# kuleshov-group/caduceus

Measured on AMD Instinct MI355X. Metric: DNA tokens/sec (whole node), hg38-style MLM pre-train step, higher is better.
Workload: dtype bf16; 1 GPU; Caduceus-PS d_model=256 n_layer=16 seqlen=131072 rcps=true MLM fwd+bwd+allreduce+AdamW, 1 seq/GPU; global_batch=1, accumulate_grad_batches=1, seq_len=131072, parallelism=dp1, params=7725312

## Files before the change

caduceus_amd/_lib.py:

```python
from __future__ import annotations

import ctypes as C
import os
import threading

import torch

HERE = os.path.dirname(os.path.abspath(__file__))
LIB_PATH = os.environ.get("CADUCEUS_AMD_LIB") or os.path.join(HERE, "libcaduceus_hip.so")

CAD_F32, CAD_BF16, CAD_F16 = 0, 1, 2
PROF_KINDS = ("scan_fwd", "scan_bwd", "conv_fwd", "conv_bwd", "add_norm_fwd", "add_norm_bwd", "embed", "lm_head", "proj")

_p = C.c_void_p
_i64 = C.c_int64
_i = C.c_int
_f = C.c_float


class EmbedArgs(C.Structure):
    _fields_ = [("ids", _p), ("comp", _p), ("weight", _p), ("out", _p), ("B", _i64), ("L", _i64), ("D", _i), ("V", _i),
                ("n_strands", _i), ("w_dtype", _i), ("out_dtype", _i)]


# ... 4 lines not shown

class AddNormArgs(C.Structure):
    _fields_ = [("x", _p), ("residual_in", _p), ("weight", _p), ("bias", _p), ("y", _p), ("residual_out", _p),
                ("rstd", _p), ("mean", _p), ("rows_per_strand", _i64), ("n_strands", _i), ("D", _i), ("eps", _f),
                ("is_rms", _i), ("swap_flip", _i), ("x_dtype", _i), ("y_dtype", _i), ("y_fp8", _p), ("y_scale", _p)]


class AddNormBwdArgs(C.Structure):
    _fields_ = [("dy", _p), ("dres_out", _p), ("sum_saved", _p), ("rstd", _p), ("mean", _p), ("weight", _p),
                ("dx", _p), ("dres_in", _p), ("dweight", _p), ("dbias", _p), ("rows_per_strand", _i64),
                ("n_strands", _i), ("D", _i), ("is_rms", _i), ("swap_flip", _i), ("x_dtype", _i), ("y_dtype", _i)]


class Conv1dArgs(C.Structure):
    _fields_ = [("x", _p), ("w", _p), ("bias", _p), ("out", _p), ("SB", _i64), ("L", _i64), ("split", _i64),
                ("E", _i), ("K", _i), ("rev_lo", _i), ("rev_hi", _i), ("dtype", _i)]


class ReduceJob(C.Structure):
    _fields_ = [("src", _p), ("dst", _p)]


class ProjTmArgs(C.Structure):
    _fields_ = [("W", _p), ("X", _p), ("X2", _p), ("out", _p), ("T", _i64), ("M", _i), ("K", _i), ("ldw", _i64), ("ldx", _i64),
                ("ldo", _i64)]


class GemmStreamArgs(C.Structure):
    _fields_ = [("A", _p), ("B", _p), ("out", _p), ("R", _i64), ("C", _i64), ("K", _i64), ("lda", _i64), ("ldb", _i64), ("ldo", _i64),
                ("nslices", _i), ("mode", _i), ("col_fastest", _i)]


class FoldF32Job(C.Structure):
    _fields_ = [("src", _p), ("dst", _p), ("n", _i64), ("stride", _i64), ("stride2", _i64), ("nparts", _i), ("nparts2", _i)]


class GemmF32Args(C.Structure):
    _fields_ = [("A", _p), ("B", _p), ("D", _p), ("addend", _p), ("M", _i64), ("N", _i64), ("K", _i64),
                ("a_rs", _i64), ("a_cs", _i64), ("b_rs", _i64), ("b_cs", _i64), ("d_rs", _i64), ("d_cs", _i64),
                ("batch", _i64), ("a_bs", _i64), ("b_bs", _i64), ("d_bs", _i64)]


class Conv1dBwdArgs(C.Structure):
    _fields_ = [("x", _p), ("w", _p), ("bias", _p), ("dout", _p), ("dx", _p), ("dw", _p), ("dbias", _p),
                ("SB", _i64), ("L", _i64), ("split", _i64), ("E", _i), ("K", _i), ("rev_lo", _i), ("rev_hi", _i),
                ("dtype", _i), ("accumulate", _i)]


class ScanArgs(C.Structure):
    _fields_ = [("u", _p), ("delta", _p), ("A", _p), ("Bm", _p), ("Cm", _p), ("D", _p), ("z", _p),
                ("delta_bias", _p), ("out", _p), ("chunk_state", _p), ("SB", _i64), ("L", _i64), ("split", _i64),
                ("E", _i), ("N", _i), ("rev_lo", _i), ("rev_hi", _i), ("dtype", _i), ("h0", _p), ("hT", _p),
                ("sum_dt", _p), ("delta_is_dt", _i), ("map_only", _i)]


class ScanBwdArgs(C.Structure):
    _fields_ = [("u", _p), ("delta", _p), ("A", _p), ("Bm", _p), ("Cm", _p), ("D", _p), ("z", _p),
                ("delta_bias", _p), ("dout", _p), ("out", _p), ("chunk_state", _p), ("du", _p), ("ddelta", _p), ("dz", _p),
                ("dA", _p), ("dB", _p), ("dC", _p), ("dD", _p), ("ddelta_bias", _p), ("SB", _i64), ("L", _i64),
                ("split", _i64), ("E", _i), ("N", _i), ("rev_lo", _i), ("rev_hi", _i), ("dtype", _i),
                ("n_partials", _i), ("dhT", _p), ("dh0", _p), ("out2", _p), ("gate_fix_list", _p), ("gate_fix_count", _p),
                ("gate_fix_dz", _p), ("delta_is_dt", _i), ("carry_only", _i), ("fold_counters", _p)]


class FoldArgs(C.Structure):
    _fields_ = [("dB_slots", _p), ("dC_slots", _p), ("dB", _p), ("dC", _p), ("counters", _p), ("abort_from", _p), ("SB", _i64),
                ("L", _i64), ("split", _i64), ("N", _i), ("n_partials", _i), ("rev_lo", _i), ("rev_hi", _i), ("dtype", _i)]
# ... 274 lines not shown
```

caduceus_amd/csrc/gemm.hip:

```cpp
#include "cad_common.h"
#include "cad_stream.h"

namespace {

#define GP_WAVES 8

template <typename TE>
__device__ __forceinline__ float gp_softplus(float x) {
    if constexpr (cad_is_bf16<TE>::value)
        return cad_softplus_lowp(x);
    else
        return cad_softplus(x);
}

#define GP_MB16 2
#define GP_NT16 32
#define GP_XFB16 1
template <int KS>
struct GpCfg {
    static constexpr int MB = KS >= 16 ? GP_MB16 : 4;
    static constexpr int MW = 16 * MB;
    static constexpr int MWG = MW * GP_WAVES;
    static constexpr int NT = KS >= 16 ? GP_NT16 : 64;
    static constexpr int ROWB = KS * 64;
// ... 1039 lines not shown
#endif

template <typename TE>
static int gemm_stream(const cad_gemm_stream_args* a, void* stream) {
    CAD_CHECK_ARG(a && a->A && a->B && a->out && (a->mode == CAD_GEMM_PARTIALS || a->mode == CAD_GEMM_OUT_T_BF16));
    if (!cad_gemm_stream_supported(a->R, a->C, a->K, a->nslices)) return CAD_ERR_UNSUPPORTED;
    CAD_CHECK_ARG(a->lda >= a->K && a->ldb >= a->C && (a->lda % 8) == 0 && (a->ldb % 8) == 0);
    CAD_CHECK_ARG((((uintptr_t)a->A | (uintptr_t)a->B) % 16) == 0);
    CAD_CHECK_ARG(a->mode == CAD_GEMM_PARTIALS || (a->nslices == 1 && a->ldo >= a->R && (a->ldo % 4) == 0 && ((uintptr_t)a->out % 8) == 0));
    CadProfScope prof(8, stream);
    const int64_t nitems = (a->R / GsCfg::RT) * (a->C / GsCfg::CT) * a->nslices;
    int64_t gx = cad_cu_count();
    if (gx > nitems) gx = nitems;
    dim3 grid((unsigned)gx), block(64 * GP_WAVES);
    if (a->mode == CAD_GEMM_PARTIALS) {
        GP_BIG_LDS((gemm_stream_kernel<CAD_GEMM_PARTIALS, TE>), GsCfg::LDS);
        CAD_LAUNCH((gemm_stream_kernel<CAD_GEMM_PARTIALS, TE>), grid, block, GsCfg::LDS, stream, *a);
    } else {
        GP_BIG_LDS((gemm_stream_kernel<CAD_GEMM_OUT_T_BF16, TE>), GsCfg::LDS);
        CAD_LAUNCH((gemm_stream_kernel<CAD_GEMM_OUT_T_BF16, TE>), grid, block, GsCfg::LDS, stream, *a);
    }
    return cad_after_launch();
}
#ifndef CAD_GEMM_TEMPLATES_ONLY
extern "C" int cad_gemm_stream(const cad_gemm_stream_args* a, void* stream) { return gemm_stream<bf16_t>(a, stream); }
#endif

#ifndef CAD_GEMM_TEMPLATES_ONLY
namespace {
struct FoldF32Jobs {
    cad_fold_f32_job j[CAD_FOLD_F32_MAX_JOBS];
    int first_block[CAD_FOLD_F32_MAX_JOBS + 1];
    int njobs;
};
#define FF_THREADS 256
__global__ __launch_bounds__(FF_THREADS) void fold_f32_multi_kernel(FoldF32Jobs jobs) {
    int ji = 0;
    while (ji + 1 < jobs.njobs && (int)blockIdx.x >= jobs.first_block[ji + 1]) ++ji;
    const cad_fold_f32_job& jb = jobs.j[ji];
    const int64_t i = ((int64_t)((int)blockIdx.x - jobs.first_block[ji]) * FF_THREADS + threadIdx.x) * 4;
    if (i >= jb.n) return;
    f32x4 acc = {0.f, 0.f, 0.f, 0.f};
    for (int j2 = 0; j2 < jb.nparts2; ++j2) {
        const float* p = jb.src + (int64_t)j2 * jb.stride2 + i;
        int k = 0;
        for (; k + 4 <= jb.nparts; k += 4) {
            const f32x4 a = *(const f32x4*)(p + (int64_t)k * jb.stride);
            const f32x4 b = *(const f32x4*)(p + (int64_t)(k + 1) * jb.stride);
            const f32x4 c = *(const f32x4*)(p + (int64_t)(k + 2) * jb.stride);
            const f32x4 d = *(const f32x4*)(p + (int64_t)(k + 3) * jb.stride);
            acc = acc + a;
            acc = acc + b;
            acc = acc + c;
            acc = acc + d;
        }
        for (; k < jb.nparts; ++k) acc = acc + *(const f32x4*)(p + (int64_t)k * jb.stride);
    }
    *(f32x4*)(jb.dst + i) = acc;
}
}

extern "C" int cad_fold_f32_multi(const cad_fold_f32_job* jobs, int njobs, void* stream) {
    CAD_CHECK_ARG(jobs && njobs >= 1 && njobs <= CAD_FOLD_F32_MAX_JOBS);
    FoldF32Jobs kj;
    kj.njobs = njobs;
    int64_t blocks = 0;
    for (int i = 0; i < njobs; ++i) {
        const cad_fold_f32_job& j = jobs[i];
        CAD_CHECK_ARG(j.src && j.dst && j.n > 0 && j.n % 4 == 0 && j.nparts >= 1 && j.nparts2 >= 1);
        CAD_CHECK_ARG(j.stride % 4 == 0 && j.stride2 % 4 == 0 && (((uintptr_t)j.src | (uintptr_t)j.dst) % 16) == 0);
        kj.j[i] = j;
        kj.first_block[i] = (int)blocks;
        blocks += (j.n / 4 + FF_THREADS - 1) / FF_THREADS;
        CAD_CHECK_ARG(blocks < (1 << 30));
    }
    for (int i = njobs; i < CAD_FOLD_F32_MAX_JOBS; ++i) kj.j[i] = jobs[0], kj.first_block[i] = (int)blocks;
    kj.first_block[njobs] = (int)blocks;
    for (int i = njobs + 1; i <= CAD_FOLD_F32_MAX_JOBS; ++i) kj.first_block[i] = (int)blocks;
    dim3 grid((unsigned)blocks), block(FF_THREADS);
    CAD_LAUNCH(fold_f32_multi_kernel, grid, block, 0, stream, kj);
    return cad_after_launch();
}
#endif
```

caduceus_amd/mixer.py:

```python
from __future__ import annotations

import ctypes as C
import os
from collections import namedtuple

import torch

from . import _lib as L
from . import ops

SetParams = namedtuple("SetParams", "conv_w conv_b W_x W_dt dt_bias A_log D")
SetSaved = namedtuple("SetSaved", "xc delta A dbc D dt_bias conv_w conv_b w_x w_dt state A_log")
SetWork = namedtuple("SetWork", "du ddelta dA dD dbias dBC npart")
Meta = namedtuple("Meta", "SB Lq split pdtypes conv_w_shapes win_dt wout_dt delta_is_dt k")
StepCache = namedtuple("StepCache", "versions w_in w_out w_x w_dt A w_inT w_outT w_xT w_dtT w_out2 w_in_fp8")
_DIRS = ((0, 1), (1, 0))


def _flatten(records):
    return [t for r in records for t in r]


def _unflatten(cls, flat, n):
    w = len(cls._fields)
    return [cls(*flat[j * w:(j + 1) * w]) for j in range(n)], flat[n * w:]


def _conv_fwd2(x, params, split, dirs):
    E, SB, Lq = x.shape
    n = len(params)
    args = (L.Conv1dArgs * n)()
    outs = []
    for i, (wf, bf) in enumerate(params):
        out = torch.empty_like(x)
        stream = L.stream_and_check(x, wf, bf, out)
        args[i] = L.Conv1dArgs(L.ptr(x), L.ptr(wf), L.ptr(bf), L.ptr(out), SB, Lq, split, E, wf.shape[1], dirs[i][0],
                               dirs[i][1], L.dtype_code(x.dtype))
        outs.append(out)
    L.check(L.get_lib().cad_conv1d_fwd_multi(args, n, stream), "cad_conv1d_fwd_multi")
    return outs


def _zeros_f32(spec, device):
    sizes = [int(torch.Size(s).numel()) for s, _ in spec.values()]
    offs = [0]
    for n in sizes:
        offs.append(offs[-1] + (n + 3) // 4 * 4)
    flat = torch.zeros((offs[-1],), dtype=torch.float32, device=device)
    return {name: flat[o:o + n].view(dt).view(s) for o, n, (name, (s, dt)) in zip(offs, sizes, spec.items())}


def _conv_bwd2(x, params, douts, dx, split, dirs, bufs=None):
    E, SB, Lq = x.shape
    n = len(params)
    args = (L.Conv1dBwdArgs * n)()
    res, slots = [], []
    for i, (wf, bf) in enumerate(params):
        if bufs is not None:
            dw, db = bufs[i]
        else:
            dw = torch.zeros_like(wf)
            db = None if bf is None else torch.zeros_like(bf)
        stream = L.stream_and_check(x, wf, bf, douts[i], dx, dw, db)
        args[i] = L.Conv1dBwdArgs(L.ptr(x), L.ptr(wf), L.ptr(bf), L.ptr(douts[i]), L.ptr(dx), L.ptr(dw), L.ptr(db), SB, Lq,
                                  split, E, wf.shape[1], dirs[i][0], dirs[i][1], L.dtype_code(x.dtype), 0)
        ns = L.get_lib().cad_conv1d_bwd_slots(C.byref(args[i]))
        ws, bs = ops.wgrad_slots(ns, dw.numel(), x.device, zero=False), (None if db is None else ops.wgrad_slots(ns, E, x.device, zero=False))
        res.append((dw, db))
        slots.append((ws, bs))
    wptr = (C.c_void_p * n)(*[ws.data_ptr() for ws, _ in slots])
    bptr = (C.c_void_p * n)(*[0 if bs is None else bs.data_ptr() for _, bs in slots])
    L.check(L.get_lib().cad_conv1d_bwd_multi_slotted(args, n, wptr, bptr, stream), "cad_conv1d_bwd_multi_slotted")
    return res


def _kchunks(T: int) -> int:
    n = 64
    while n > 1 and (T % n != 0 or T // n < 1024):
        n //= 2
    return n


# ... 12 lines not shown


def _own_wgrad_chunked_ok(X: torch.Tensor, M: int) -> bool:
    K, T = X.shape
    return K > 512 and K % 512 == 0 and ops.proj_wgrad_only_supported(X, M, 512, T)


def _own_wgrad_chunked(X: torch.Tensor, Y: torch.Tensor) -> torch.Tensor:
    K = X.shape[0]
    return torch.cat([ops.proj_wgrad_only(X[h:h + 512], Y) for h in range(0, K, 512)], dim=1)


def _wgrad_cm_tm(a_cm: torch.Tensor, b_tm: torch.Tensor) -> torch.Tensor:
    M, T = a_cm.shape
    if _OWN_GEMM:
        own = ops.wgrad_cm_tm(a_cm, b_tm)
        if own is not None:
            return own
    if a_cm.dtype in (torch.float32, torch.float16):
        return ops.mm_f32(a_cm.float(), b_tm.float())
    n = _kchunks(T)
    if n == 1:
        return ops.mm(a_cm, b_tm).float()
    Kc = T // n
    return torch.sum(ops.bmm(a_cm.view(M, n, Kc).permute(1, 0, 2), b_tm.view(n, Kc, -1)), dim=0, dtype=torch.float32)


_FUSED_WGRAD = True
_OWN_DWX = True
_OWN_OUT_PROJ = True
_OWN_GEMM = True
_STREAM_PROJ_D512 = True
_GLUE_FOLD = True
_FP8_IN_PROJ = os.environ.get("CADUCEUS_AMD_FP8_PROJ", "0") == "1"
_STREAM_FOLD = os.environ.get("CADUCEUS_AMD_STREAM_FOLD", "1") != "0"
_STREAM_FOLD_MIN_CHUNKS = 16


CAPTURE_XPROJ_OPERANDS = None


def set_fp8_in_proj(on: bool) -> None:
    global _FP8_IN_PROJ
    _FP8_IN_PROJ = bool(on)
    ops.FP8_ACTIVATIONS = _FP8_IN_PROJ


ops.FP8_ACTIVATIONS = _FP8_IN_PROJ


def prepare_step_cache(pairs, act: torch.dtype) -> None:
    if not pairs:
        return
    src, dst, alog, owners = [], [], [], []
    kinds = ("in", "out", "x", "dt")
    plist = [{"in": [mf.in_proj.weight], "out": [mf.out_proj.weight], "x": [mf.x_proj.weight, mr.x_proj.weight],
              "dt": [mf.dt_proj.weight, mr.dt_proj.weight]} for mf, mr in pairs]
    stacked = {}
    for kd in kinds:
        shapes = {tuple(p.shape) for pl in plist for p in pl[kd]}
        n = sum(len(pl[kd]) for pl in plist)
        if len(shapes) == 1:
            stacked[kd] = torch.empty((n,) + next(iter(shapes)), dtype=act, device=plist[0][kd][0].device)
    cursor = {kd: 0 for kd in kinds}

    def alloc(kd, p):
        if kd in stacked:
            v = stacked[kd][cursor[kd]]
            cursor[kd] += 1
            return v
        return torch.empty(p.shape, dtype=act, device=p.device)

    order = ("in", "out", "x", "dt", "x", "dt")
    for (mf, mr), pl in zip(pairs, plist):
        ps = [pl["in"][0], pl["out"][0], pl["x"][0], pl["dt"][0], pl["x"][1], pl["dt"][1]]
        out = [alloc(kd, p) for kd, p in zip(order, ps)]
        src += [p.detach() for p in ps]
        dst += out
        alog += [mf.A_log.detach().float(), mr.A_log.detach().float()]
        owners.append((mf, ps + [mf.A_log, mr.A_log], out))
    torch._foreach_copy_(dst, src)
    need_in_T = "in" in stacked and (_dx2d_is_streamed() or _in_proj_is_streamed(stacked["in"].shape[2], act))
    trans = {kd: stacked[kd].transpose(1, 2).contiguous() for kd in ("out", "x", "dt") + (("in",) if need_in_T else ()) if kd in stacked}
    cursor = {kd: 0 for kd in kinds}

    def transposed(kd, w):
        if kd in trans:
            v = trans[kd][cursor[kd]]
            cursor[kd] += 1
            return v
        return w.t().contiguous()

    wTs = []
    for mf, ps, (w_in, w_out, w_x_f, w_dt_f, w_x_r, w_dt_r) in owners:
        w_outT, w_x_fT, w_dt_fT, w_x_rT, w_dt_rT = [transposed(kd, w) for kd, w in zip(order[1:], (w_out, w_x_f, w_dt_f, w_x_r, w_dt_r))]
        wTs.append(dict(w_outT=w_outT, w_xT=(w_x_fT, w_x_rT), w_dtT=(w_dt_fT, w_dt_rT), w_inT=transposed("in", w_in) if need_in_T else None))
    negA = torch._foreach_exp(alog)
    torch._foreach_neg_(negA)
    for (mf, ps, (w_in, w_out, w_x_f, w_dt_f, w_x_r, w_dt_r)), wT, A_f, A_r in zip(owners, wTs, negA[0::2], negA[1::2]):
        w_out2 = torch.cat([w_out, w_out], 1) if _out_proj_is_streamed(w_out.shape[0]) else None
        w_in_fp8 = None
        if _FP8_IN_PROJ and act == torch.bfloat16 and ops.fp8_proj_supported(w_in, w_in.shape[1]):
            w_in_fp8 = ops.quant_weight_fp8(mf.in_proj.weight)
        mf._cad_step_cache = StepCache(versions=[(id(p), p._version) for p in ps], w_in=w_in, w_out=w_out, w_x=(w_x_f, w_x_r),
                                       w_dt=(w_dt_f, w_dt_r), A=(A_f, A_r), w_out2=w_out2, w_in_fp8=w_in_fp8, **wT)


def _cached(mf, params):
    c = getattr(mf, "_cad_step_cache", None)
    if c is None or c.versions != [(id(p), p._version) for p in params]:
        return None
    return c


def _transposed(cache, field, w, i=None):
    wT = None if cache is None else getattr(cache, field)
    if wT is not None and i is not None:
        wT = wT[i]
    return w.t().contiguous() if wT is None else wT


def _in_proj_is_streamed(Dm: int, act) -> bool:
    return _STREAM_PROJ_D512 and Dm > 256 and act == torch.bfloat16


def _in_proj(x2d, W_in, w_in, cache, fp8_act):
    T, Dm = x2d.shape
    if _FP8_IN_PROJ and x2d.dtype == torch.bfloat16 and ops.fp8_proj_supported(x2d, Dm):
        wq, sw = cache.w_in_fp8 if (cache and cache.w_in_fp8 is not None) else ops.quant_weight_fp8(W_in)
        xq, sx = (fp8_act[0].view(T, Dm), fp8_act[1]) if fp8_act is not None else ops.quant_rows_fp8(x2d)
        return ops.proj_wxT_fp8(wq, sw, xq, sx)
    xz = None
    if _in_proj_is_streamed(Dm, x2d.dtype):
        xz = ops.gemm_out_t(x2d, _transposed(cache, "w_inT", w_in))
    if xz is None and ops.proj_supported(x2d, Dm):
        xz = ops.proj_wxT(w_in, x2d)
    if xz is None:
        xz = ops.mm(w_in, x2d.t())
# ... 40 lines not shown

def _out_proj(w_out, ycat, cache):
    Dm, E = w_out.shape
    T = ycat.shape[1]
    if _OWN_OUT_PROJ and ops.proj_xTw_supported(ycat, Dm, E, T):
        return ops.proj_xTw(w_out, ycat[:E], ycat[E:])
    out2d = None
    if _STREAM_PROJ_D512 and ycat.dtype == torch.bfloat16:
        w_out2 = cache.w_out2 if cache else None
        out2d = ops.proj_xTw_stream(w_out2 if w_out2 is not None else torch.cat([w_out, w_out], 1), ycat)
    if out2d is None:
        out2d = ops.mm(ycat.t(), torch.cat([w_out, w_out], 1).t())
    return out2d


def _d_y(dout2d, w_out, cache):
    Dm = dout2d.shape[1]
    dy = None
    if _STREAM_PROJ_D512 and Dm > 256 and dout2d.dtype == torch.bfloat16:
        dy = ops.gemm_out_t(dout2d, w_out)
    if dy is None and ops.proj_supported(dout2d, Dm):
        dy = ops.proj_wxT(_transposed(cache, "w_outT", w_out), dout2d)
    if dy is None:
        dy = ops.mm(w_out.t(), dout2d.t())
    return dy


def _dW_out(ycat, dout2d, glue):
    E, Dm = ycat.shape[0] // 2, dout2d.shape[1]
    part = ops.wgrad_cm_tm(ycat, dout2d, return_partials=True) if (_GLUE_FOLD and _OWN_GEMM) else None
    if part is None:
        dW_cat = _wgrad_cm_tm(ycat, dout2d)
        return (dW_cat[:E] + dW_cat[E:]).t()
    dW_out_ED = torch.empty((E, Dm), dtype=torch.float32, device=ycat.device)
    glue.append((part, dW_out_ED, E * Dm, part.shape[0], 2 * E * Dm, 2, E * Dm))
    return dW_out_ED.t()


def _scan_bwd(sets, xz, ycat, dy, seg_P, meta):
    lib = L.get_lib()
    SB, Lq, split, k, act, dev = meta.SB, meta.Lq, meta.split, meta.k, xz.dtype, xz.device
    E = xz.shape[0] // 2
    z = xz[E:]
    dxz = torch.empty_like(xz)
    spec = {}
    for i, s in enumerate(sets):
        spec.update({("dA", i): (s.A.shape, torch.float32), ("dD", i): (s.D.shape, torch.float32),
                     ("dbias", i): (s.dt_bias.shape, torch.float32), ("conv_dw", i): (s.conv_w.shape, torch.float32),
                     ("conv_db", i): (s.conv_b.shape if s.conv_b is not None else (0,), torch.float32)})
    spec.update({("fix_cnt", i): ((1,), torch.int32) for i in range(2)})
    N = sets[0].A.shape[1]
    npart = lib.cad_scan_bwd_partials(E)
    nch = max(1, (Lq // k) // int(lib.cad_scan_bwd_chunk_len()))
    stream_fold = (_STREAM_FOLD and sets[1].A.shape[1] == N and ops.fold_stream_supported(N, npart, Lq // k, act)
                   and nch >= _STREAM_FOLD_MIN_CHUNKS and npart * SB * k * 2 <= 4 * ops._cu_count()
                   and ops.fold_side_available(dev))
    if stream_fold:
        nci = (int(lib.cad_scan_bwd_fold_counter_ints(SB * k, Lq // k)) + 3) // 4 * 4
        spec.update({"fold_counters": ((2, nci), torch.int32), "give_ups": ((2, SB * k, npart), torch.int32)})
    zero = _zeros_f32(spec, dev)
    n_fix = lib.cad_scan_gate_fix_entries(E, SB, Lq)
    fix_list = [torch.empty((n_fix,), dtype=torch.int64, device=dev) for _ in range(2)]
    args = (L.ScanBwdArgs * 2)()
    work = []
    for i, (s, y) in enumerate(zip(sets, ycat.view(2, E, SB, Lq))):
        N = s.A.shape[1]
        R = s.dbc.shape[0] - 2 * N
        np_i = lib.cad_scan_bwd_partials(E)
        w = SetWork(torch.empty_like(s.xc), torch.empty_like(s.xc), zero["dA", i], zero["dD", i], zero["dbias", i],
                    torch.empty((2, np_i, N, SB, Lq), dtype=ops.scan_slot_dtype(act), device=dev), np_i)
        dz = dxz[E:] if i == 0 else None
        Bm, Cm = s.dbc[R:R + N], s.dbc[R + N:]
        args[i], stream = ops.scan_bwd_args(E, SB, Lq, N, split, _DIRS[i], act, w.npart, k=k, delta_is_dt=meta.delta_is_dt[i], u=s.xc,
                                            delta=s.delta, A=s.A, Bm=Bm, Cm=Cm, D=s.D, z=z, delta_bias=s.dt_bias, dout=dy, out=y,
                                            chunk_state=s.state, du=w.du, ddelta=w.ddelta, dz=dz, dA=w.dA, dB=w.dBC[0], dC=w.dBC[1],
                                            dD=w.dD, ddelta_bias=w.dbias, out2=ycat[E:] if i == 0 else None, gate_fix_list=fix_list[i],
                                            gate_fix_count=zero["fix_cnt", i], gate_fix_dz=dxz[E:],
                                            fold_counters=zero["fold_counters"][i] if stream_fold else None)
        work.append(w)
    ddbcs = [torch.empty_like(s.dbc) for s in sets]
    rows = []
    for s, w, ddbc in zip(sets, work, ddbcs):
        N = s.A.shape[1]
        R = s.dbc.shape[0] - 2 * N
        rows.append((*map(L.ptr, w.dBC), L.ptr(ddbc[R:R + N]), L.ptr(ddbc[R + N:])))
    launch_scan = lambda: ops.scan_bwd_launch(lib, args, 2, stream, k, seg_P, _DIRS, split)
    if stream_fold:
        fargs = (L.FoldArgs * 2)()
        for i, (s, w) in enumerate(zip(sets, work)):
            fargs[i] = L.FoldArgs(*rows[i], L.ptr(zero["fold_counters"][i]), L.ptr(zero["give_ups"][i]), SB * k, Lq // k, split * k,
                                  s.A.shape[1], w.npart, *_DIRS[i], L.dtype_code(act))
        _keep = ops.fold_behind_scan(lib, fargs, 2, dev, launch_scan, give_ups=zero["give_ups"])
    else:
        _keep = launch_scan()
    L.check(lib.cad_scan_bwd_gate_fix(args, 2, stream), "cad_scan_bwd_gate_fix")
    if not stream_fold:
        jobs = (L.ReduceJob * 4)(*[L.ReduceJob(src, dst) for dB_s, dC_s, dB, dC in rows for src, dst in ((dB_s, dB), (dC_s, dC))])
        assert work[0].npart == work[1].npart and sets[0].A.shape[1] == sets[1].A.shape[1], "one fold launch: both sets share depth and d_state"
        L.check(lib.cad_reduce_partials_multi(jobs, 4, work[0].npart, sets[0].A.shape[1] * SB * Lq, L.dtype_code(act), stream),
                "cad_reduce_partials_multi")
    return dxz, work, ddbcs, [(zero["conv_dw", i], zero["conv_db", i] if s.conv_b is not None else None) for i, s in enumerate(sets)]


def _d_dt_lr(s, w, ddbc, i, cache, slots):
    (E, T), R = s.xc.shape, s.w_dt.shape[1]
    ddelta, dt_lr, out = w.ddelta, s.dbc[:R], ddbc[:R]
    if _FUSED_WGRAD and ops.proj_wx_wgrad_supported(ddelta, R, E, T):
        if "dt" not in slots:
            slots["dt"] = ops.wgrad_partials(T, E, R, ddelta.device, nsets=2)
        ops.proj_wx_wgrad(_transposed(cache, "w_dtT", s.w_dt, i), ddelta, dt_lr, out=out, part=slots["dt"][i])
        return None
    if ops.proj_wx_supported(ddelta, E, T, M=R):
        ops.proj_wx(_transposed(cache, "w_dtT", s.w_dt, i), ddelta, out=out)
    else:
        ops.mm(s.w_dt.t(), ddelta, out=out)
    if _OWN_DWX and _own_wgrad_chunked_ok(ddelta, R):
        return _own_wgrad_chunked(ddelta, dt_lr).t()
    return _wgrad_cm_cm(ddelta, dt_lr)


def _dW_x(s, ddbc, i, slots):
    xc, (E, T), M = s.xc, s.xc.shape, ddbc.shape[0]
    if _OWN_DWX and ops.proj_wgrad_only_supported(xc, M, E, T):
        if "x" not in slots:
            slots["x"] = ops.wgrad_partials(T, E, M, xc.device, nsets=2)
        ops.proj_wgrad_only(xc, ddbc, part=slots["x"][i])
        return None
    if _OWN_DWX and _own_wgrad_chunked_ok(xc, M):
        return _own_wgrad_chunked(xc, ddbc)
    return _wgrad_cm_cm(ddbc, xc)


def _d_xc(s, du, ddbc, i, cache):
    M, T = ddbc.shape
# ... 2 lines not shown
    elif du.dtype == torch.float32:
        ops.mm_f32(s.w_x.t(), ddbc, out=du, addend=du)
    elif du.dtype == torch.float16:
        du.copy_(ops.mm_f32(s.w_x.t().float(), ddbc.float(), addend=du.float()))
    else:
        du.addmm_(s.w_x.t(), ddbc)


def _dx2d_is_streamed() -> bool:
    return _OWN_GEMM


def _d_x2d(dxz, w_in, cache):
    dx2d = ops.proj_xTw_stream(_transposed(cache, "w_inT", w_in), dxz) if _dx2d_is_streamed() else None
    return ops.mm(dxz.t(), w_in) if dx2d is None else dx2d


def _dW_in_partials(dxz, x2d, glue):
    part = ops.wgrad_cm_tm(dxz, x2d, return_partials=True) if (_GLUE_FOLD and _OWN_GEMM) else None
    if part is None:
        return None
    dW_in = torch.empty((dxz.shape[0], x2d.shape[1]), dtype=torch.float32, device=x2d.device)
    glue.append((part, dW_in, dW_in.numel(), part.shape[0], dW_in.numel(), 1, 0))
    return dW_in


def _wgrad_slot_sums(slots, glue):
    if not _GLUE_FOLD:
        return {name: wg.sum(dim=1) for name, wg in slots.items()}
    sums = {}
    for name in ("dt", "x"):
        if name in slots:
            _, P, K, M = slots[name].shape
            sums[name] = torch.empty((2, K, M), dtype=torch.float32, device=slots[name].device)
            glue += [(src, dst, K * M, P, K * M, 1, 0) for src, dst in zip(slots[name], sums[name])]
    return sums


class BiMambaMixerFn(torch.autograd.Function):

    @staticmethod
    def forward(ctx, x2d, SB, Lq, split, cache, fp8_act, W_in, W_out, *ps):
        act = x2d.dtype
        T = x2d.shape[0]
        E = W_in.shape[0] // 2
        params, _ = _unflatten(SetParams, ps, 2)
        if cache is not None and cache.w_in.dtype != act:
            cache = None
        w_in = cache.w_in if cache else W_in.to(act)
        w_out = cache.w_out if cache else W_out.to(act)
        xz = _in_proj(x2d, W_in, w_in, cache, fp8_act).view(2 * E, SB, Lq)
        x, z = xz[:E], xz[E:]
        cparams = [(p.conv_w.float().reshape(E, -1).contiguous(), None if p.conv_b is None else p.conv_b.float().contiguous())
                   for p in params]
        xcs = [xc.view(E, T) for xc in _conv_fwd2(x, cparams, split, _DIRS)]
        sets, delta_is_dt = [], []
        for i, (p, xc, (conv_w, conv_b)) in enumerate(zip(params, xcs, cparams)):
            w_x, w_dt = (cache.w_x[i], cache.w_dt[i]) if cache else (p.W_x.to(act), p.W_dt.to(act))
            dbc = _x_proj(w_x, xc)
            dt_bias = p.dt_bias.float().contiguous()
            delta, fused = _dt_proj(w_dt, dbc[:w_dt.shape[1]], dt_bias)
            A = cache.A[i] if cache else -torch.exp(p.A_log.float())
            sets.append(SetSaved(xc, delta, A, dbc, p.D.float().contiguous(), dt_bias, conv_w, conv_b, w_x, w_dt, None, p.A_log))
            delta_is_dt.append(fused)
        k = ops.lsplit_factor(E, SB, Lq, 2)
        ycat = torch.empty((2 * E, SB, Lq), dtype=act, device=x2d.device)
        sets, seg_P = _scan_fwd(sets, z, ycat, delta_is_dt, split, k)
        out2d = _out_proj(w_out, ycat.view(2 * E, T), cache)
        ctx.cache = cache
        ctx.save_for_backward(x2d, xz, w_in, w_out, ycat, *_flatten(sets), *seg_P)
        ctx.meta = Meta(SB, Lq, split, [SetParams(*(None if t is None else t.dtype for t in p)) for p in params],
                        [p.conv_w.shape for p in params], W_in.dtype, W_out.dtype, tuple(delta_is_dt), k)
        return out2d

    @staticmethod
    def backward(ctx, dout2d):
        x2d, xz, w_in, w_out, ycat, *rest = ctx.saved_tensors
        sets, seg_P = _unflatten(SetSaved, rest, 2)
        meta, cache = ctx.meta, ctx.cache
        T = x2d.shape[0]
        E = xz.shape[0] // 2
        dout2d = dout2d.contiguous()
        glue = []
        slots = {}
        dy = _d_y(dout2d, w_out, cache)
        dW_out = _dW_out(ycat.view(2 * E, T), dout2d, glue)
        dxz, work, ddbcs, conv_bufs = _scan_bwd(sets, xz, ycat, dy, seg_P, meta)
        part = []
        for i, (s, w, ddbc) in enumerate(zip(sets, work, ddbcs)):
            dW_dt = _d_dt_lr(s, w, ddbc, i, cache, slots)
            dW_x = _dW_x(s, ddbc, i, slots)
            _d_xc(s, w.du, ddbc, i, cache)
            part.append((dW_x, dW_dt, w.dA * s.A))
        if CAPTURE_XPROJ_OPERANDS is not None:
            CAPTURE_XPROJ_OPERANDS.append({"ddbc": [d.clone() for d in ddbcs], "xc": [s.xc.clone() for s in sets]})
        conv_g = _conv_bwd2(xz[:E], [(s.conv_w, s.conv_b) for s in sets], [w.du for w in work], dxz[:E], meta.split, _DIRS,
                            bufs=conv_bufs)
        sums = _wgrad_slot_sums(slots, glue)
        dx2d = _d_x2d(dxz.view(2 * E, T), w_in, cache)
        dW_in = _dW_in_partials(dxz.view(2 * E, T), x2d, glue)
        if glue:
            ops.fold_f32(glue)
        if "x" in sums:
            sums["x"] = sums["x"].transpose(1, 2).contiguous()
        grads = []
        for i, (dt, (dwc, dbc_conv), (dW_x, dW_dt, dA_log), w) in enumerate(zip(meta.pdtypes, conv_g, part, work)):
            dW_x = sums["x"][i] if dW_x is None else dW_x
            dW_dt = sums["dt"][i] if dW_dt is None else dW_dt
            grads += SetParams(conv_w=dwc.reshape(meta.conv_w_shapes[i]).to(dt.conv_w),
                               conv_b=None if dbc_conv is None else dbc_conv.to(dt.conv_b), W_x=dW_x.to(dt.W_x), W_dt=dW_dt.to(dt.W_dt),
                               dt_bias=w.dbias.to(dt.dt_bias), A_log=dA_log.to(dt.A_log), D=w.dD.to(dt.D))
        if dW_in is None:
            dW_in = _wgrad_cm_tm(dxz.view(2 * E, T), x2d)
        return (dx2d, None, None, None, None, None, dW_in.to(meta.win_dt), dW_out.to(meta.wout_dt), *grads)


def can_use(mamba_fwd, mamba_rev, strategy) -> bool:
    if mamba_rev is None or (strategy or "add") != "add":
        return False
    tied = (mamba_rev.in_proj.weight is mamba_fwd.in_proj.weight and mamba_rev.out_proj.weight is mamba_fwd.out_proj.weight)
    no_bias = mamba_fwd.in_proj.bias is None and mamba_fwd.out_proj.bias is None
    same = mamba_fwd.d_state == mamba_rev.d_state and mamba_fwd.dt_rank == mamba_rev.dt_rank
    return bool(tied and no_bias and same)


def bimamba_mixer(hn: torch.Tensor, mamba_fwd, mamba_rev, split: int) -> torch.Tensor:
    S, B, Lq, Dm = hn.shape
    ps = _flatten(SetParams(m.conv1d.weight, m.conv1d.bias, m.x_proj.weight, m.dt_proj.weight, m.dt_proj.bias, m.A_log, m.D)
                  for m in (mamba_fwd, mamba_rev))
    cache = _cached(mamba_fwd, [mamba_fwd.in_proj.weight, mamba_fwd.out_proj.weight, mamba_fwd.x_proj.weight,
                                mamba_fwd.dt_proj.weight, mamba_rev.x_proj.weight, mamba_rev.dt_proj.weight,
                                mamba_fwd.A_log, mamba_rev.A_log])
    fp8_act = ops.fp8_operand_of(hn) if _FP8_IN_PROJ else None
    out = BiMambaMixerFn.apply(hn.reshape(S * B * Lq, Dm), S * B, Lq, split, cache, fp8_act, mamba_fwd.in_proj.weight,
                               mamba_fwd.out_proj.weight, *ps)
    return out.view(S, B, Lq, Dm)
```

caduceus_amd/ops.py:

```python
from __future__ import annotations

import ctypes as C
import math
import os
from typing import Optional, Tuple

import torch

from . import _lib as L


def _zeros_like_f32(t, shape=None):
    return torch.zeros(t.shape if shape is None else shape, dtype=torch.float32, device=t.device)


class _Embed(torch.autograd.Function):
    @staticmethod
    def forward(ctx, ids, weight, comp, n_strands, out_dtype):
        ids = ids.contiguous()
        w = weight.contiguous()
        B, Lq = ids.shape
        V, D = w.shape
        out = torch.empty((n_strands, B, Lq, D), dtype=out_dtype, device=w.device)
        stream = L.stream_and_check(ids, w, comp, out)
# ... 956 lines not shown

def proj_xTw_supported(X: torch.Tensor, M: int, K: int, T: int) -> bool:
    return X.dtype in _MFMA_DTYPES and bool(L.get_lib().cad_proj_xTw_supported(int(M), int(K), int(T)))


def proj_xTw(W: torch.Tensor, X: torch.Tensor, X2: Optional[torch.Tensor] = None, out: Optional[torch.Tensor] = None) -> torch.Tensor:
    M, K = W.shape
    T = X.shape[1]
    _same_mfma_dtype(W, X, X2, out)
    if out is None:
        out = torch.empty((T, M), dtype=X.dtype, device=X.device)
    stream = L.stream_and_check(W, X, X2, out, contiguous=False)
    assert W.stride(1) == 1 and X.stride(1) == 1 and out.stride(1) == 1 and (X2 is None or (X2.stride() == X.stride() and X2.shape == X.shape))
    a = L.ProjTmArgs(L.ptr(W), L.ptr(X), L.ptr(X2), L.ptr(out), T, M, K, W.stride(0), X.stride(0), out.stride(0))
    L.check(_proj_fn("cad_proj_xTw", X.dtype)(C.byref(a), stream), "cad_proj_xTw")
    return out


GEMM_PARTIALS, GEMM_OUT_T_BF16 = 0, 1


def gemm_stream_slices(R: int, Cc: int, K: int) -> int:
    if R % 256 or Cc % 256 or R < 256 or Cc < 256:
        return 0
    n = max(1, _cu_count() // ((R // 256) * (Cc // 256)))
    while n > 1 and (K % (32 * n) != 0):
        n -= 1
    return n if K % (32 * n) == 0 else 0


def fold_f32(jobs) -> None:
    arr = (L.FoldF32Job * len(jobs))()
    tensors = []
    for q, (src, dst, n, nparts, stride, nparts2, stride2) in enumerate(jobs):
        if src.dtype != torch.float32 or dst.dtype != torch.float32 or not dst.is_contiguous() or dst.numel() != n:
            raise ValueError("fold_f32: fp32 tensors, dst contiguous with n elements")
        arr[q] = L.FoldF32Job(L.ptr(src), L.ptr(dst), n, stride, stride2, nparts, nparts2)
        tensors += [src, dst]
    stream = L.stream_and_check(*tensors, contiguous=False)
    L.check(L.get_lib().cad_fold_f32_multi(arr, len(jobs), stream), "cad_fold_f32_multi")


def wgrad_cm_tm(a_cm: torch.Tensor, b_tm: torch.Tensor, return_partials: bool = False) -> Optional[torch.Tensor]:
    M, T = a_cm.shape
    N = b_tm.shape[1]
    if a_cm.dtype not in _MFMA_DTYPES or b_tm.dtype != a_cm.dtype or a_cm.stride(1) != 1 or b_tm.stride(1) != 1:
        return None
    if a_cm.stride(0) % 8 or b_tm.stride(0) % 8 or a_cm.data_ptr() % 16 or b_tm.data_ptr() % 16:
        return None
    n = gemm_stream_slices(M, N, T)
    if n == 0 or not L.get_lib().cad_gemm_stream_supported(M, N, T, n):
        return None
    part = torch.empty((n, M, N), dtype=torch.float32, device=a_cm.device)
    stream = L.stream_and_check(a_cm, b_tm, part, contiguous=False)
    a = L.GemmStreamArgs(L.ptr(a_cm), L.ptr(b_tm), L.ptr(part), M, N, T, a_cm.stride(0), b_tm.stride(0), 0, n, GEMM_PARTIALS)
    L.check(_proj_fn("cad_gemm_stream", a_cm.dtype)(C.byref(a), stream), "cad_gemm_stream")
    if return_partials:
        return part
    return part[0] if n == 1 else part.sum(0)


def gemm_out_t(A: torch.Tensor, B: torch.Tensor, col_fastest: bool = True) -> Optional[torch.Tensor]:
    return proj_xTw_stream(A, B, col_fastest=col_fastest)


def proj_xTw_stream(Wt: torch.Tensor, X: torch.Tensor, col_fastest: bool = False) -> Optional[torch.Tensor]:
    M, K = Wt.shape
    T = X.shape[1]
    if X.dtype not in _MFMA_DTYPES or Wt.dtype != X.dtype or Wt.stride(1) != 1 or X.stride(1) != 1:
        return None
    if Wt.stride(0) % 8 or X.stride(0) % 8 or Wt.data_ptr() % 16 or X.data_ptr() % 16:
# ... 230 lines not shown
```

include/caduceus_hip.h:

```cpp
#ifndef CADUCEUS_HIP_H
#define CADUCEUS_HIP_H

#include <stddef.h>
#include <stdint.h>

#ifdef __cplusplus
extern "C" {
#endif

typedef enum { CAD_OK = 0, CAD_ERR_BAD_ARG = 1, CAD_ERR_UNSUPPORTED = 2, CAD_ERR_LAUNCH = 3 } cad_status;
typedef enum { CAD_F32 = 0, CAD_BF16 = 1, CAD_F16 = 2 } cad_dtype;

const char* cad_version(void);
const char* cad_status_string(int status);
int cad_is_device_build(void);
int cad_debug_set_cu_count(int n);

typedef struct {
    const int64_t* ids;
    const int64_t* comp;
    const void* weight;
    void* out;
    int64_t B, L;
    int D, V, n_strands;
// ... 203 lines not shown
int cad_proj_wx_wgrad_f16(const cad_proj_args* a, void* stream);
int cad_proj_wx_wgrad_supported(int M, int K, int64_t T);
int cad_proj_wgrad_only_supported(int M, int K, int64_t T);
int cad_proj_wx_wgrad_partials(int64_t T);

typedef struct {
    const void* W;
    const void* X;
    const void* X2;
    void* out;
    int64_t T;
    int M, K;
    int64_t ldw, ldx, ldo;
} cad_proj_tm_args;
int cad_proj_xTw(const cad_proj_tm_args* a, void* stream);
int cad_proj_xTw_f16(const cad_proj_tm_args* a, void* stream);
int cad_proj_xTw_supported(int M, int K, int64_t T);

#define CAD_GEMM_PARTIALS 0
#define CAD_GEMM_OUT_T_BF16 1
typedef struct {
    const void* A;
    const void* B;
    void* out;
    int64_t R, C, K;
    int64_t lda, ldb, ldo;
    int nslices;
    int mode;
    int col_fastest;
} cad_gemm_stream_args;
int cad_gemm_stream(const cad_gemm_stream_args* a, void* stream);
int cad_gemm_stream_f16(const cad_gemm_stream_args* a, void* stream);

#define CAD_FOLD_F32_MAX_JOBS 8
typedef struct {
    const float* src;
    float* dst;
    int64_t n;
    int64_t stride, stride2;
    int nparts, nparts2;
} cad_fold_f32_job;
int cad_fold_f32_multi(const cad_fold_f32_job* jobs, int njobs, void* stream);

typedef struct {
    const float* A;
    const float* B;
    float* D;
    const float* addend;
    int64_t M, N, K;
    int64_t a_rs, a_cs, b_rs, b_cs, d_rs, d_cs;
    int64_t batch, a_bs, b_bs, d_bs;
} cad_gemm_f32_args;
int cad_gemm_f32(const cad_gemm_f32_args* a, void* stream);
int cad_gemm_b16(const cad_gemm_f32_args* a, int out_f32, void* stream);
int cad_gemm_stream_supported(int64_t R, int64_t C, int64_t K, int nslices);

typedef struct {
    const void* x;
    void* q;
    float* scale;
    int64_t T;
    int K;
    int64_t ldx, ldq;
    int dtype;
} cad_quant_fp8_args;
int cad_quant_rows_fp8(const cad_quant_fp8_args* a, void* stream);
typedef struct {
    const void* Wq;
    const void* Xq;
    const float* sw;
    const float* sx;
    void* out;
    int64_t T;
// ... 198 lines not shown
```

Baseline: 1.122 million tokens/s.

## Fold per-channel grad finishing and transposes into the multi-job fold kernel

```diff
diff --git a/caduceus_amd/_lib.py b/caduceus_amd/_lib.py
--- a/caduceus_amd/_lib.py
+++ b/caduceus_amd/_lib.py
@@ -60,7 +60,8 @@
 
 
 class FoldF32Job(C.Structure):
-    _fields_ = [("src", _p), ("dst", _p), ("n", _i64), ("stride", _i64), ("stride2", _i64), ("nparts", _i), ("nparts2", _i)]
+    _fields_ = [("src", _p), ("dst", _p), ("n", _i64), ("stride", _i64), ("stride2", _i64), ("nparts", _i), ("nparts2", _i),
+                ("mul", _p), ("cols", _i64), ("dst_rs", _i64), ("dst_cs", _i64)]
 
 
 class GemmF32Args(C.Structure):
diff --git a/caduceus_amd/csrc/gemm.hip b/caduceus_amd/csrc/gemm.hip
--- a/caduceus_amd/csrc/gemm.hip
+++ b/caduceus_amd/csrc/gemm.hip
@@ -1095,6 +1095,7 @@
     cad_fold_f32_job j[CAD_FOLD_F32_MAX_JOBS];
     int first_block[CAD_FOLD_F32_MAX_JOBS + 1];
     int njobs;
+    unsigned vec_src, vec_dst;
 };
 #define FF_THREADS 256
 __global__ __launch_bounds__(FF_THREADS) void fold_f32_multi_kernel(FoldF32Jobs jobs) {
@@ -1103,23 +1104,55 @@
     const cad_fold_f32_job& jb = jobs.j[ji];
     const int64_t i = ((int64_t)((int)blockIdx.x - jobs.first_block[ji]) * FF_THREADS + threadIdx.x) * 4;
     if (i >= jb.n) return;
+    const int ne = jb.n - i < 4 ? (int)(jb.n - i) : 4;
     f32x4 acc = {0.f, 0.f, 0.f, 0.f};
-    for (int j2 = 0; j2 < jb.nparts2; ++j2) {
-        const float* p = jb.src + (int64_t)j2 * jb.stride2 + i;
-        int k = 0;
-        for (; k + 4 <= jb.nparts; k += 4) {
-            const f32x4 a = *(const f32x4*)(p + (int64_t)k * jb.stride);
-            const f32x4 b = *(const f32x4*)(p + (int64_t)(k + 1) * jb.stride);
-            const f32x4 c = *(const f32x4*)(p + (int64_t)(k + 2) * jb.stride);
-            const f32x4 d = *(const f32x4*)(p + (int64_t)(k + 3) * jb.stride);
-            acc = acc + a;
-            acc = acc + b;
-            acc = acc + c;
-            acc = acc + d;
-        }
-        for (; k < jb.nparts; ++k) acc = acc + *(const f32x4*)(p + (int64_t)k * jb.stride);
-    }
-    *(f32x4*)(jb.dst + i) = acc;
+    if (jb.nparts == 1 && jb.nparts2 == 1) {
+        if ((jobs.vec_src >> ji) & 1u) {
+            acc = *(const f32x4*)(jb.src + i);
+        } else {
+            for (int e = 0; e < ne; ++e) acc[e] = jb.src[i + e];
+        }
+    } else if ((jobs.vec_src >> ji) & 1u) {
+        for (int j2 = 0; j2 < jb.nparts2; ++j2) {
+            const float* p = jb.src + (int64_t)j2 * jb.stride2 + i;
+            int k = 0;
+            for (; k + 4 <= jb.nparts; k += 4) {
+                const f32x4 a = *(const f32x4*)(p + (int64_t)k * jb.stride);
+                const f32x4 b = *(const f32x4*)(p + (int64_t)(k + 1) * jb.stride);
+                const f32x4 c = *(const f32x4*)(p + (int64_t)(k + 2) * jb.stride);
+                const f32x4 d = *(const f32x4*)(p + (int64_t)(k + 3) * jb.stride);
+                acc = acc + a;
+                acc = acc + b;
+                acc = acc + c;
+                acc = acc + d;
+            }
+            for (; k < jb.nparts; ++k) acc = acc + *(const f32x4*)(p + (int64_t)k * jb.stride);
+        }
+    } else {
+        for (int j2 = 0; j2 < jb.nparts2; ++j2) {
+            const float* p = jb.src + (int64_t)j2 * jb.stride2 + i;
+            for (int k = 0; k < jb.nparts; ++k)
+                for (int e = 0; e < ne; ++e) acc[e] = acc[e] + p[(int64_t)k * jb.stride + e];
+        }
+    }
+    const bool vdst = (jobs.vec_dst >> ji) & 1u;
+    if (jb.mul) {
+        if (vdst) {
+            acc = acc * *(const f32x4*)(jb.mul + i);
+        } else {
+            for (int e = 0; e < ne; ++e) acc[e] = acc[e] * jb.mul[i + e];
+        }
+    }
+    if (vdst) {
+        *(f32x4*)(jb.dst + i) = acc;
+    } else if (jb.cols == 0) {
+        for (int e = 0; e < ne; ++e) jb.dst[i + e] = acc[e];
+    } else {
+        for (int e = 0; e < ne; ++e) {
+            const int64_t r = (i + e) / jb.cols, c = (i + e) - r * jb.cols;
+            jb.dst[r * jb.dst_rs + c * jb.dst_cs] = acc[e];
+        }
+    }
 }
 }
 
@@ -1127,14 +1160,19 @@
     CAD_CHECK_ARG(jobs && njobs >= 1 && njobs <= CAD_FOLD_F32_MAX_JOBS);
     FoldF32Jobs kj;
     kj.njobs = njobs;
+    kj.vec_src = kj.vec_dst = 0;
     int64_t blocks = 0;
     for (int i = 0; i < njobs; ++i) {
         const cad_fold_f32_job& j = jobs[i];
-        CAD_CHECK_ARG(j.src && j.dst && j.n > 0 && j.n % 4 == 0 && j.nparts >= 1 && j.nparts2 >= 1);
-        CAD_CHECK_ARG(j.stride % 4 == 0 && j.stride2 % 4 == 0 && (((uintptr_t)j.src | (uintptr_t)j.dst) % 16) == 0);
+        CAD_CHECK_ARG(j.src && j.dst && j.n > 0 && j.nparts >= 1 && j.nparts2 >= 1);
+        CAD_CHECK_ARG((((uintptr_t)j.src | (uintptr_t)j.dst | (uintptr_t)j.mul) % 4) == 0);
+        CAD_CHECK_ARG(j.cols >= 0 && (j.cols == 0 || (j.n % j.cols == 0 && j.dst_rs >= 0 && j.dst_cs >= 0)));
+        const bool contiguous = j.cols == 0 || (j.dst_cs == 1 && j.dst_rs == j.cols) || (j.cols == j.n && j.dst_cs == 1);
+        if (j.n % 4 == 0 && j.stride % 4 == 0 && j.stride2 % 4 == 0 && (uintptr_t)j.src % 16 == 0) kj.vec_src |= 1u << i;
+        if (j.n % 4 == 0 && contiguous && (((uintptr_t)j.dst | (uintptr_t)j.mul) % 16) == 0) kj.vec_dst |= 1u << i;
         kj.j[i] = j;
         kj.first_block[i] = (int)blocks;
-        blocks += (j.n / 4 + FF_THREADS - 1) / FF_THREADS;
+        blocks += ((j.n + 3) / 4 + FF_THREADS - 1) / FF_THREADS;
         CAD_CHECK_ARG(blocks < (1 << 30));
     }
     for (int i = njobs; i < CAD_FOLD_F32_MAX_JOBS; ++i) kj.j[i] = jobs[0], kj.first_block[i] = (int)blocks;
diff --git a/caduceus_amd/mixer.py b/caduceus_amd/mixer.py
--- a/caduceus_amd/mixer.py
+++ b/caduceus_amd/mixer.py
@@ -13,7 +13,7 @@
 SetSaved = namedtuple("SetSaved", "xc delta A dbc D dt_bias conv_w conv_b w_x w_dt state A_log")
 SetWork = namedtuple("SetWork", "du ddelta dA dD dbias dBC npart")
 Meta = namedtuple("Meta", "SB Lq split pdtypes conv_w_shapes win_dt wout_dt delta_is_dt k")
-StepCache = namedtuple("StepCache", "versions w_in w_out w_x w_dt A w_inT w_outT w_xT w_dtT w_out2 w_in_fp8")
+StepCache = namedtuple("StepCache", "versions w_in w_out w_x w_dt A w_inT w_outT w_xT w_dtT w_out2 w_in_fp8 zeros")
 _DIRS = ((0, 1), (1, 0))
 
 
@@ -41,13 +41,43 @@
     return outs
 
 
-def _zeros_f32(spec, device):
+def _zeros_f32(spec, device, pool=None):
     sizes = [int(torch.Size(s).numel()) for s, _ in spec.values()]
     offs = [0]
     for n in sizes:
         offs.append(offs[-1] + (n + 3) // 4 * 4)
-    flat = torch.zeros((offs[-1],), dtype=torch.float32, device=device)
+    flat = None if pool is None else pool.take(offs[-1], device)
+    if flat is None:
+        flat = torch.zeros((offs[-1],), dtype=torch.float32, device=device)
     return {name: flat[o:o + n].view(dt).view(s) for o, n, (name, (s, dt)) in zip(offs, sizes, spec.items())}
+
+
+class _StepZeros:
+
+    def __init__(self, nlayers: int):
+        self.nlayers, self.flat, self.per, self.taken = nlayers, None, 0, set()
+
+    def slot(self, index: int):
+        return _StepZerosSlot(self, index)
+
+
+class _StepZerosSlot:
+    def __init__(self, pool, index):
+        self.pool, self.index = pool, index
+
+    def take(self, nfloats: int, device):
+        p = self.pool
+        if p.flat is None and not p.taken:
+            p.per = (nfloats + 63) // 64 * 64
+            p.flat = torch.zeros((p.nlayers * p.per,), dtype=torch.float32, device=device)
+        if self.index in p.taken or nfloats > p.per or p.flat is None or p.flat.device != device:
+            return None
+        p.taken.add(self.index)
+        if len(p.taken) == p.nlayers:
+            flat, p.flat = p.flat, None
+        else:
+            flat = p.flat
+        return flat[self.index * p.per:self.index * p.per + nfloats]
 
 
 def _conv_bwd2(x, params, douts, dx, split, dirs, bufs=None):
@@ -126,6 +156,7 @@
 _OWN_GEMM = True
 _STREAM_PROJ_D512 = True
 _GLUE_FOLD = True
+_GLUE_FINISH = True
 _FP8_IN_PROJ = os.environ.get("CADUCEUS_AMD_FP8_PROJ", "0") == "1"
 _STREAM_FOLD = os.environ.get("CADUCEUS_AMD_STREAM_FOLD", "1") != "0"
 _STREAM_FOLD_MIN_CHUNKS = 16
@@ -191,13 +222,15 @@
         wTs.append(dict(w_outT=w_outT, w_xT=(w_x_fT, w_x_rT), w_dtT=(w_dt_fT, w_dt_rT), w_inT=transposed("in", w_in) if need_in_T else None))
     negA = torch._foreach_exp(alog)
     torch._foreach_neg_(negA)
-    for (mf, ps, (w_in, w_out, w_x_f, w_dt_f, w_x_r, w_dt_r)), wT, A_f, A_r in zip(owners, wTs, negA[0::2], negA[1::2]):
+    zeros = _StepZeros(len(owners))
+    for li, ((mf, ps, (w_in, w_out, w_x_f, w_dt_f, w_x_r, w_dt_r)), wT, A_f, A_r) in enumerate(zip(owners, wTs, negA[0::2], negA[1::2])):
         w_out2 = torch.cat([w_out, w_out], 1) if _out_proj_is_streamed(w_out.shape[0]) else None
         w_in_fp8 = None
         if _FP8_IN_PROJ and act == torch.bfloat16 and ops.fp8_proj_supported(w_in, w_in.shape[1]):
             w_in_fp8 = ops.quant_weight_fp8(mf.in_proj.weight)
         mf._cad_step_cache = StepCache(versions=[(id(p), p._version) for p in ps], w_in=w_in, w_out=w_out, w_x=(w_x_f, w_x_r),
-                                       w_dt=(w_dt_f, w_dt_r), A=(A_f, A_r), w_out2=w_out2, w_in_fp8=w_in_fp8, **wT)
+                                       w_dt=(w_dt_f, w_dt_r), A=(A_f, A_r), w_out2=w_out2, w_in_fp8=w_in_fp8,
+                                       zeros=zeros.slot(li) if _GLUE_FINISH else None, **wT)
 
 
 def _cached(mf, params):
@@ -304,12 +337,16 @@
     if part is None:
         dW_cat = _wgrad_cm_tm(ycat, dout2d)
         return (dW_cat[:E] + dW_cat[E:]).t()
+    if _GLUE_FINISH:
+        dW_out = torch.empty((Dm, E), dtype=torch.float32, device=ycat.device)
+        glue.append((part, dW_out.t(), E * Dm, part.shape[0], 2 * E * Dm, 2, E * Dm))
+        return dW_out
     dW_out_ED = torch.empty((E, Dm), dtype=torch.float32, device=ycat.device)
     glue.append((part, dW_out_ED, E * Dm, part.shape[0], 2 * E * Dm, 2, E * Dm))
     return dW_out_ED.t()
 
 
-def _scan_bwd(sets, xz, ycat, dy, seg_P, meta):
+def _scan_bwd(sets, xz, ycat, dy, seg_P, meta, cache=None):
     lib = L.get_lib()
     SB, Lq, split, k, act, dev = meta.SB, meta.Lq, meta.split, meta.k, xz.dtype, xz.device
     E = xz.shape[0] // 2
@@ -318,8 +355,10 @@
     spec = {}
     for i, s in enumerate(sets):
         spec.update({("dA", i): (s.A.shape, torch.float32), ("dD", i): (s.D.shape, torch.float32),
-                     ("dbias", i): (s.dt_bias.shape, torch.float32), ("conv_dw", i): (s.conv_w.shape, torch.float32),
-                     ("conv_db", i): (s.conv_b.shape if s.conv_b is not None else (0,), torch.float32)})
+                     ("dbias", i): (s.dt_bias.shape, torch.float32)})
+        if not _GLUE_FINISH:
+            spec.update({("conv_dw", i): (s.conv_w.shape, torch.float32),
+                         ("conv_db", i): (s.conv_b.shape if s.conv_b is not None else (0,), torch.float32)})
     spec.update({("fix_cnt", i): ((1,), torch.int32) for i in range(2)})
     N = sets[0].A.shape[1]
     npart = lib.cad_scan_bwd_partials(E)
@@ -330,7 +369,7 @@
     if stream_fold:
         nci = (int(lib.cad_scan_bwd_fold_counter_ints(SB * k, Lq // k)) + 3) // 4 * 4
         spec.update({"fold_counters": ((2, nci), torch.int32), "give_ups": ((2, SB * k, npart), torch.int32)})
-    zero = _zeros_f32(spec, dev)
+    zero = _zeros_f32(spec, dev, cache.zeros if (cache is not None and _GLUE_FINISH) else None)
     n_fix = lib.cad_scan_gate_fix_entries(E, SB, Lq)
     fix_list = [torch.empty((n_fix,), dtype=torch.int64, device=dev) for _ in range(2)]
     args = (L.ScanBwdArgs * 2)()
@@ -371,7 +410,11 @@
         assert work[0].npart == work[1].npart and sets[0].A.shape[1] == sets[1].A.shape[1], "one fold launch: both sets share depth and d_state"
         L.check(lib.cad_reduce_partials_multi(jobs, 4, work[0].npart, sets[0].A.shape[1] * SB * Lq, L.dtype_code(act), stream),
                 "cad_reduce_partials_multi")
-    return dxz, work, ddbcs, [(zero["conv_dw", i], zero["conv_db", i] if s.conv_b is not None else None) for i, s in enumerate(sets)]
+    if _GLUE_FINISH:
+        conv_bufs = [(torch.empty_like(s.conv_w), None if s.conv_b is None else torch.empty_like(s.conv_b)) for s in sets]
+    else:
+        conv_bufs = [(zero["conv_dw", i], zero["conv_db", i] if s.conv_b is not None else None) for i, s in enumerate(sets)]
+    return dxz, work, ddbcs, conv_bufs
 
 
 def _d_dt_lr(s, w, ddbc, i, cache, slots):
@@ -440,6 +483,11 @@
     for name in ("dt", "x"):
         if name in slots:
             _, P, K, M = slots[name].shape
+            if _GLUE_FINISH:
+                own = [torch.empty((M, K) if name == "x" else (K, M), dtype=torch.float32, device=slots[name].device) for _ in range(2)]
+                glue += [(src, dst.t() if name == "x" else dst, K * M, P, K * M, 1, 0) for src, dst in zip(slots[name], own)]
+                sums[name] = own
+                continue
             sums[name] = torch.empty((2, K, M), dtype=torch.float32, device=slots[name].device)
             glue += [(src, dst, K * M, P, K * M, 1, 0) for src, dst in zip(slots[name], sums[name])]
     return sums
@@ -493,13 +541,22 @@
         slots = {}
         dy = _d_y(dout2d, w_out, cache)
         dW_out = _dW_out(ycat.view(2 * E, T), dout2d, glue)
-        dxz, work, ddbcs, conv_bufs = _scan_bwd(sets, xz, ycat, dy, seg_P, meta)
-        part = []
+        dxz, work, ddbcs, conv_bufs = _scan_bwd(sets, xz, ycat, dy, seg_P, meta, cache)
+        finish = _GLUE_FINISH and bool(glue)
+        part, chan = [], []
         for i, (s, w, ddbc) in enumerate(zip(sets, work, ddbcs)):
             dW_dt = _d_dt_lr(s, w, ddbc, i, cache, slots)
             dW_x = _dW_x(s, ddbc, i, slots)
             _d_xc(s, w.du, ddbc, i, cache)
-            part.append((dW_x, dW_dt, w.dA * s.A))
+            if finish:
+                dA_log, dD, dbias = torch.empty_like(s.A), torch.empty_like(s.D), torch.empty_like(s.dt_bias)
+                glue += [(w.dA, dA_log, dA_log.numel(), 1, dA_log.numel(), 1, 0, s.A), (w.dD, dD, dD.numel(), 1, dD.numel(), 1, 0),
+                         (w.dbias, dbias, dbias.numel(), 1, dbias.numel(), 1, 0)]
+            else:
+                dA_log = w.dA * s.A
+                dD, dbias = (w.dD.clone(), w.dbias.clone()) if _GLUE_FINISH else (w.dD, w.dbias)
+            part.append((dW_x, dW_dt, dA_log))
+            chan.append((dD, dbias))
         if CAPTURE_XPROJ_OPERANDS is not None:
             CAPTURE_XPROJ_OPERANDS.append({"ddbc": [d.clone() for d in ddbcs], "xc": [s.xc.clone() for s in sets]})
         conv_g = _conv_bwd2(xz[:E], [(s.conv_w, s.conv_b) for s in sets], [w.du for w in work], dxz[:E], meta.split, _DIRS,
@@ -509,15 +566,15 @@
         dW_in = _dW_in_partials(dxz.view(2 * E, T), x2d, glue)
         if glue:
             ops.fold_f32(glue)
-        if "x" in sums:
+        if "x" in sums and torch.is_tensor(sums["x"]):
             sums["x"] = sums["x"].transpose(1, 2).contiguous()
         grads = []
-        for i, (dt, (dwc, dbc_conv), (dW_x, dW_dt, dA_log), w) in enumerate(zip(meta.pdtypes, conv_g, part, work)):
+        for i, (dt, (dwc, dbc_conv), (dW_x, dW_dt, dA_log), (dD, dbias)) in enumerate(zip(meta.pdtypes, conv_g, part, chan)):
             dW_x = sums["x"][i] if dW_x is None else dW_x
             dW_dt = sums["dt"][i] if dW_dt is None else dW_dt
             grads += SetParams(conv_w=dwc.reshape(meta.conv_w_shapes[i]).to(dt.conv_w),
                                conv_b=None if dbc_conv is None else dbc_conv.to(dt.conv_b), W_x=dW_x.to(dt.W_x), W_dt=dW_dt.to(dt.W_dt),
-                               dt_bias=w.dbias.to(dt.dt_bias), A_log=dA_log.to(dt.A_log), D=w.dD.to(dt.D))
+                               dt_bias=dbias.to(dt.dt_bias), A_log=dA_log.to(dt.A_log), D=dD.to(dt.D))
         if dW_in is None:
             dW_in = _wgrad_cm_tm(dxz.view(2 * E, T), x2d)
         return (dx2d, None, None, None, None, None, dW_in.to(meta.win_dt), dW_out.to(meta.wout_dt), *grads)
diff --git a/caduceus_amd/ops.py b/caduceus_amd/ops.py
--- a/caduceus_amd/ops.py
+++ b/caduceus_amd/ops.py
@@ -1012,11 +1012,15 @@
 def fold_f32(jobs) -> None:
     arr = (L.FoldF32Job * len(jobs))()
     tensors = []
-    for q, (src, dst, n, nparts, stride, nparts2, stride2) in enumerate(jobs):
-        if src.dtype != torch.float32 or dst.dtype != torch.float32 or not dst.is_contiguous() or dst.numel() != n:
-            raise ValueError("fold_f32: fp32 tensors, dst contiguous with n elements")
-        arr[q] = L.FoldF32Job(L.ptr(src), L.ptr(dst), n, stride, stride2, nparts, nparts2)
-        tensors += [src, dst]
+    for q, (src, dst, n, nparts, stride, nparts2, stride2, *more) in enumerate(jobs):
+        mul = more[0] if more else None
+        if src.dtype != torch.float32 or dst.dtype != torch.float32 or dst.numel() != n or not (dst.is_contiguous() or dst.dim() == 2):
+            raise ValueError("fold_f32: fp32 tensors, dst with n elements, contiguous or a 2-D view")
+        if mul is not None and (mul.dtype != torch.float32 or mul.numel() != n or not mul.is_contiguous()):
+            raise ValueError("fold_f32: mul fp32, contiguous, n elements")
+        cols, rs, cs = (0, 0, 0) if dst.is_contiguous() else (dst.shape[1], *dst.stride())
+        arr[q] = L.FoldF32Job(L.ptr(src), L.ptr(dst), n, stride, stride2, nparts, nparts2, L.ptr(mul), cols, rs, cs)
+        tensors += [src, dst, mul]
     stream = L.stream_and_check(*tensors, contiguous=False)
     L.check(L.get_lib().cad_fold_f32_multi(arr, len(jobs), stream), "cad_fold_f32_multi")
 
diff --git a/include/caduceus_hip.h b/include/caduceus_hip.h
--- a/include/caduceus_hip.h
+++ b/include/caduceus_hip.h
@@ -259,13 +259,15 @@
 int cad_gemm_stream(const cad_gemm_stream_args* a, void* stream);
 int cad_gemm_stream_f16(const cad_gemm_stream_args* a, void* stream);
 
-#define CAD_FOLD_F32_MAX_JOBS 8
+#define CAD_FOLD_F32_MAX_JOBS 16
 typedef struct {
     const float* src;
     float* dst;
     int64_t n;
     int64_t stride, stride2;
     int nparts, nparts2;
+    const float* mul;
+    int64_t cols, dst_rs, dst_cs;
 } cad_fold_f32_job;
 int cad_fold_f32_multi(const cad_fold_f32_job* jobs, int njobs, void* stream);
 
```

Measured after the change: 1.125 million tokens/s, median of 3. Within noise of the previous version (+0.3%).
